# simon-donike/NIR-GAN

Measured on AMD Instinct MI355X. Metric: 256x256 RGB tiles/sec (G+D fwd+bwd+step), higher is better.
Workload: dtype f32 (3xbf16 split, 6 products, f32 accumulate) for the contractions with 32-channel runs incl. the Winograd plane GEMMs; exact f32 MFMA for the first / last layers; f32 everywhere else; 1 GPU; configs[1]: 6-block ResnetGenerator + 3-layer PatchGAN, bs=16/GPU, 256x256, GAN+L1, padding=0, fp32-equivalent MFMA (three bf16 terms, six products); global_batch=16, parallelism=dp1

## Files before the change

nir-gan_amd/csrc/igemm_wgrad.hip:

```cpp
#include "igemm_tiles.h"
#include "igemm_tile256.h"
#include "igemm_x3.h"
#include <cstdlib>

namespace {

template <int TN, int PREC = 0>
__global__ __launch_bounds__(256, 2) void wgrad_igemm_kernel(const ng::WgradParams p) {
    __shared__ __attribute__((aligned(16))) char st0[32 * (TN + 128) * 4];
    __shared__ __attribute__((aligned(16))) char st1[32 * (TN + 128) * 4];
    ng::wgrad_tile<TN, PREC>(p, blockIdx.x, st0, st1);
}

__global__ __launch_bounds__(256, 2) void wgrad_persist_kernel(const ng::WgradParams p) {
    __shared__ __attribute__((aligned(16))) char lds[65536];
    ng::wgrad_persist(p, blockIdx.x, gridDim.x, lds);
}

__global__ __launch_bounds__(256, 2) void wgrad_igemm16_kernel(const ng::WgradParams p) {
    __shared__ __attribute__((aligned(16))) char st0[32768];
    __shared__ __attribute__((aligned(16))) char st1[32768];
    ng::wgrad_tile16(p, blockIdx.x, st0, st1);
}


template <int PREC = 0, bool WB16 = false, bool AB16 = false, bool TW16 = false>
__global__ __launch_bounds__(256, 2) void conv_wgrad_pair_kernel(const ng::ConvParams cp, const ng::WgradParams wp, const int conv_blocks) {
    __shared__ __attribute__((aligned(16))) char st0[32768];
    __shared__ __attribute__((aligned(16))) char st1[32768];
    if (int(blockIdx.x) < conv_blocks)
        ng::conv_tile<128, PREC, WB16, AB16>(cp, blockIdx.x, st0, st1);
    else if constexpr (TW16)
        ng::wgrad_tile16(wp, int(blockIdx.x) - conv_blocks, st0, st1);
    else
        ng::wgrad_tile<128, PREC>(wp, int(blockIdx.x) - conv_blocks, st0, st1);
}

__global__ __launch_bounds__(512, 2) void wgrad_igemm256_kernel(const ng::WgradParams p, const int units) {
    __shared__ __attribute__((aligned(16))) char lds[ng::T256_LDS];
    bool again = false;
    for (int u = ng_xcd_remap(blockIdx.x, gridDim.x); u < units; u += gridDim.x) {
        if (again) ng::t256_bar();
        ng::wgrad_tile256(p, u, lds);
        again = true;
    }
}

__global__ __launch_bounds__(512, 2) void conv_wgrad_pair256_kernel(const ng::ConvParams cp, const ng::WgradParams wp, const int conv_wgs,
                                                                     const int conv_tiles, const int wgrad_units) {
    __shared__ __attribute__((aligned(16))) char lds[ng::T256_LDS];
    bool again = false;
    if (int(blockIdx.x) < conv_wgs) {
        for (int t = ng_xcd_remap(blockIdx.x, conv_wgs); t < conv_tiles; t += conv_wgs) {
            if (again) ng::t256_bar();
            ng::conv_tile256(cp, t, lds);
            again = true;
        }
    } else {
        const int y = int(gridDim.x) - conv_wgs;
        for (int u = ng_xcd_remap(int(blockIdx.x) - conv_wgs, y); u < wgrad_units; u += y) {
            if (again) ng::t256_bar();
            ng::wgrad_tile256(wp, u, lds);
            again = true;
        }
    }
}

template <int TN>
__global__ __launch_bounds__(512, 2) void wgrad_x3_kernel(const ng::WgradParams p, const int units) {
    __shared__ __attribute__((aligned(16))) char sP0[3 * 32 * TN * 2];
    __shared__ __attribute__((aligned(16))) char sP1[3 * 32 * TN * 2];
    __shared__ __attribute__((aligned(16))) char sQ0[3 * 32 * 256];
    __shared__ __attribute__((aligned(16))) char sQ1[3 * 32 * 256];
    for (int u = ng_xcd_remap(blockIdx.x, gridDim.x); u < units; u += gridDim.x) {
        ng::wgrad_tile_x3<TN>(p, u, sP0, sP1, sQ0, sQ1);
        __syncthreads();
    }
}

__global__ __launch_bounds__(256) void reduce_rows_kernel(const float* __restrict__ slabs, int nsplit, int N, int K,
                                                          const int32_t* __restrict__ map, float* __restrict__ dst,
                                                          int64_t dst_elems, int dst_row_stride, int accumulate, int row0) {
    __shared__ f32x4 part[4][64];
    const int lane = threadIdx.x & 63, grp = threadIdx.x >> 6;
    const int k4 = (blockIdx.x * 64 + lane) * 4;
    const int n = blockIdx.y;
    const size_t total = size_t(N) * K;
    f32x4 s = {0.f, 0.f, 0.f, 0.f};
    if (k4 < K) {
        const float* src = slabs + size_t(row0 + n) * K + k4;
        f32x4 s1 = {0.f, 0.f, 0.f, 0.f}, s2 = {0.f, 0.f, 0.f, 0.f}, s3 = {0.f, 0.f, 0.f, 0.f};
        int sp = grp;
        for (; sp + 12 < nsplit; sp += 16) {
            s += *reinterpret_cast<const f32x4*>(src + sp * total);
            s1 += *reinterpret_cast<const f32x4*>(src + (sp + 4) * total);
            s2 += *reinterpret_cast<const f32x4*>(src + (sp + 8) * total);
            s3 += *reinterpret_cast<const f32x4*>(src + (sp + 12) * total);
        }
        for (; sp < nsplit; sp += 4) s += *reinterpret_cast<const f32x4*>(src + sp * total);
        s = (s + s1) + (s2 + s3);
    }
    part[grp][lane] = s;
    __syncthreads();
    if (grp != 0 || k4 >= K) return;
    s = (part[0][lane] + part[1][lane]) + (part[2][lane] + part[3][lane]);
#pragma unroll
    for (int j = 0; j < 4; ++j) {
        const int mk = map[k4 + j];
        if (mk < 0) continue;
        const int64_t o = int64_t(n) * dst_row_stride + mk;
        if (o < dst_elems) dst[o] = accumulate ? dst[o] + s[j] : s[j];
    }
}

__global__ __launch_bounds__(256) void reduce_rows_batch_kernel(const long long* __restrict__ jobs, int njobs) {
    __shared__ f32x4 part[4][256];
    __shared__ float tile[64 * 16];
    int j = 0;
    for (int i = 1; i < njobs; ++i)
        if (int(blockIdx.x) >= int(jobs[i * 10 + 8])) j = i;
    const long long* J = jobs + j * 10;
    const float* slabs = reinterpret_cast<const float*>(J[0]);
    float* dst = reinterpret_cast<float*>(J[1]);
    const int32_t* map = reinterpret_cast<const int32_t*>(J[2]);
    const int nsplit = int(J[3]), N = int(J[4]), K = int(J[5]);
    const long long dst_elems = J[6];
    const int dst_row_stride = int(J[7] & 0xffffffffll), accumulate = int(J[7] >> 32);
    const int taps = int(J[9]);
    const int local = int(blockIdx.x) - int(J[8]);
    const int lane = threadIdx.x & 63, grp = threadIdx.x >> 6;
    const size_t total = size_t(N) * K;
    auto sum_splits = [&](const float* src) {
        f32x4 s = {0.f, 0.f, 0.f, 0.f}, s1 = {0.f, 0.f, 0.f, 0.f}, s2 = {0.f, 0.f, 0.f, 0.f}, s3 = {0.f, 0.f, 0.f, 0.f};
        int sp = grp;
        for (; sp + 12 < nsplit; sp += 16) {
            s += *reinterpret_cast<const f32x4*>(src + sp * total);
            s1 += *reinterpret_cast<const f32x4*>(src + (sp + 4) * total);
            s2 += *reinterpret_cast<const f32x4*>(src + (sp + 8) * total);
            s3 += *reinterpret_cast<const f32x4*>(src + (sp + 12) * total);
        }
        for (; sp < nsplit; sp += 4) s += *reinterpret_cast<const f32x4*>(src + sp * total);
        return (s + s1) + (s2 + s3);
    };
    if (taps > 0) {
        const int cin = K / taps, cb = cin >> 6;
        const int n = local / cb, c0 = (local - n * cb) << 6;
        const int nf = taps * 16;
        for (int f = lane; f < nf; f += 64) {
            const int t = f >> 4, q = f & 15;
            part[grp][f] = sum_splits(slabs + size_t(n) * K + t * cin + c0 + q * 4);
        }
        __syncthreads();
        for (int f = threadIdx.x; f < nf; f += 256) {
            const int t = f >> 4, q = f & 15;
            const f32x4 v = (part[0][f] + part[1][f]) + (part[2][f] + part[3][f]);
#pragma unroll
            for (int e = 0; e < 4; ++e) tile[(q * 4 + e) * taps + t] = v[e];
        }
        __syncthreads();
        float* drow = dst + (long long)n * dst_row_stride + (long long)c0 * taps;
        for (int i = threadIdx.x; i < 64 * taps; i += 256) drow[i] = accumulate ? drow[i] + tile[i] : tile[i];
        return;
    }
    const int kblocks = (K + 255) / 256;
    const int n = local / kblocks, kb = local - n * kblocks;
    const int k4 = (kb * 64 + lane) * 4;
    f32x4 s = {0.f, 0.f, 0.f, 0.f};
    if (k4 < K) s = sum_splits(slabs + size_t(n) * K + k4);
    part[grp][lane] = s;
    __syncthreads();
    if (grp != 0 || k4 >= K) return;
    s = (part[0][lane] + part[1][lane]) + (part[2][lane] + part[3][lane]);
#pragma unroll
    for (int q = 0; q < 4; ++q) {
        const int mk = map[k4 + q];
        if (mk < 0) continue;
        const long long o = (long long)n * dst_row_stride + mk;
        if (o < dst_elems) dst[o] = accumulate ? dst[o] + s[q] : s[q];
    }
}

typedef __bf16 bf16x4_t __attribute__((ext_vector_type(4)));

__device__ __forceinline__ void pack_store(float* dst, size_t elem, f32x4 v, int bf16) {
    if (bf16) *reinterpret_cast<bf16x4_t*>(reinterpret_cast<unsigned short*>(dst) + elem) = __builtin_convertvector(v, bf16x4_t);
    else *reinterpret_cast<f32x4*>(dst + elem) = v;
}

__global__ __launch_bounds__(256) void pack_rows_kernel(const float* __restrict__ src, int64_t src_elems, int src_row_stride,
                                                        const int32_t* __restrict__ map, float* __restrict__ dst, int N, int K, int bf16) {
    const int k4 = (blockIdx.x * 256 + threadIdx.x) * 4;
    const int n = blockIdx.y;
    if (k4 >= K) return;
    f32x4 v = {0.f, 0.f, 0.f, 0.f};
#pragma unroll
    for (int j = 0; j < 4; ++j) {
        const int mk = map[k4 + j];
        if (mk >= 0) {
            const int64_t o = int64_t(n) * src_row_stride + mk;
            if (o < src_elems) v[j] = src[o];
        }
    }
    pack_store(dst, size_t(n) * K + k4, v, bf16);
}

__global__ __launch_bounds__(256) void pack_rows_batch_kernel(const long long* __restrict__ jobs, int njobs) {
    int j = 0;
    for (int i = 1; i < njobs; ++i)
        if (int(blockIdx.x) >= int(jobs[i * 10 + 7])) j = i;
    const long long* J = jobs + j * 10;
    const float* src = reinterpret_cast<const float*>(J[0]);
    float* dst = reinterpret_cast<float*>(J[1]);
    const int32_t* map = reinterpret_cast<const int32_t*>(J[2]);
    const long long src_elems = J[3];
    const int K = int(J[5]), stride = int(J[6] & 0xffffffffll), bf16 = int(J[6] >> 32);
    const int kblocks = (K + 1023) / 1024;
    const int local = int(blockIdx.x) - int(J[7]);
    const int n = local / kblocks, kb = local - n * kblocks;
    const int k4 = (kb * 256 + threadIdx.x) * 4;
    if (k4 >= K) return;
    f32x4 v = {0.f, 0.f, 0.f, 0.f};
#pragma unroll
    for (int q = 0; q < 4; ++q) {
        const int mk = map[k4 + q];
        if (mk >= 0) {
            const long long o = (long long)n * stride + mk;
            if (o < src_elems) v[q] = src[o];
        }
    }
    pack_store(dst, size_t(n) * K + k4, v, bf16);
    if (J[8] != 0) {
        unsigned short* w3 = reinterpret_cast<unsigned short*>(J[8]) + size_t(n) * K + k4;
        const long long plane = J[9];
        typedef unsigned u32x2 __attribute__((ext_vector_type(2)));
        u32x2 h, m, l;
#pragma unroll
        for (int i = 0; i < 2; ++i) {
            const float x0 = v[2 * i], x1 = v[2 * i + 1];
            h[i] = ng::x3_pk(x0, x1);
            const float r0 = x0 - __builtin_bit_cast(float, h[i] << 16), r1 = x1 - __builtin_bit_cast(float, h[i] & 0xffff0000u);
            m[i] = ng::x3_pk(r0, r1);
            l[i] = ng::x3_pk(r0 - __builtin_bit_cast(float, m[i] << 16), r1 - __builtin_bit_cast(float, m[i] & 0xffff0000u));
        }
        *reinterpret_cast<u32x2*>(w3) = h;
        *reinterpret_cast<u32x2*>(w3 + plane) = m;
        *reinterpret_cast<u32x2*>(w3 + 2 * plane) = l;
    }
}

}


static int ng_cu_count() {
    static int cus = 0;
    if (cus == 0) {
        int dev = 0, n = 0;
        if (hipGetDevice(&dev) != hipSuccess || hipDeviceGetAttribute(&n, hipDeviceAttributeMultiprocessorCount, dev) != hipSuccess || n <= 0) n = 256;
        cus = n;
    }
    return cus;
}

static int pair256_split(const int G, const int conv_tiles, const int conv_nk, const int units, const int unit_nk) {
    int best = 1;
    long long best_cost = -1;
    for (int x = 1; x < G; ++x) {
        const long long c = (long long)((conv_tiles + x - 1) / x) * (conv_nk * 10 + 65), w = (long long)((units + (G - x) - 1) / (G - x)) * (unit_nk * 12 + 40);
        const long long cost = c > w ? c : w;
        if (best_cost < 0 || cost < best_cost) { best_cost = cost; best = x; }
    }
    return best;
}

enum WgradKernel { WGRAD_X3_TN256, WGRAD_X3_TN128, WGRAD_TILE256, WGRAD_PERSIST, WGRAD_TILE16, WGRAD_TILE_TN128, WGRAD_TILE_TN64 };
static const char* const WGRAD_KERNEL_NAMES[] = {"wgrad_x3_kernel<256>", "wgrad_x3_kernel<128>", "wgrad_igemm256_kernel", "wgrad_persist_kernel",
                                                 "wgrad_igemm16_kernel", "wgrad_igemm_kernel<128>", "wgrad_igemm_kernel<64>"};
struct WgradRoute { WgradKernel k; int units, grid; };
static WgradRoute wgrad_route(ng::WgradParams& p, const int algo) {
    const int G = ng_cu_count();
    if (p.prec == 3) {
        if (ng::wgrad_x3_ok(p)) {
            const int tn = ng::wgrad_x3_tn(p);
            const int units = (p.N / tn) * ((p.K + 127) >> 7) * p.nsplit * p.nplanes;
            return {tn == 256 ? WGRAD_X3_TN256 : WGRAD_X3_TN128, units, units < G ? units : G};
        }
        p.prec = 0;
    }
    if (algo == 0 && ng::wgrad_tile256_ok(p)) {
        const int units = (p.N >> 8) * (p.K >> 8) * p.nsplit;
        return {WGRAD_TILE256, units, units < G ? units : G};
    }
    const int tiles = p.ntiles_n * p.ntiles_k * p.nsplit * p.nplanes;
    if (ng::wgrad_persist_ok(p) && ng::wgrad_matrix_form(p) && tiles > 512 && algo != NIRGAN_WGRAD_ONE_UNIT) return {WGRAD_PERSIST, tiles, 512};
    if (p.pq_bf16) return {WGRAD_TILE16, tiles, tiles};
    return {p.N > 64 ? WGRAD_TILE_TN128 : WGRAD_TILE_TN64, tiles, tiles};
}

extern "C" int nirgan_wgrad_igemm(const nirgan_wgrad_desc* d, void* stream) {
    ng::WgradParams p;
    const int rc = ng::build_wgrad_params(d, p);
    if (rc != NIRGAN_OK) return rc;
    hipStream_t st = static_cast<hipStream_t>(stream);
    const WgradRoute r = wgrad_route(p, d->algo);
    const dim3 grid(r.grid);
    switch (r.k) {
        case WGRAD_X3_TN256: hipLaunchKernelGGL(wgrad_x3_kernel<256>, grid, dim3(512), 0, st, p, r.units); return nirgan_check_launch("wgrad_igemm (three-term split tile)");
        case WGRAD_X3_TN128: hipLaunchKernelGGL(wgrad_x3_kernel<128>, grid, dim3(512), 0, st, p, r.units); return nirgan_check_launch("wgrad_igemm (three-term split tile)");
        case WGRAD_TILE256: hipLaunchKernelGGL(wgrad_igemm256_kernel, grid, dim3(512), 0, st, p, r.units); return nirgan_check_launch("wgrad_igemm (256 x 256 tile)");
        case WGRAD_PERSIST: hipLaunchKernelGGL(wgrad_persist_kernel, grid, dim3(256), 0, st, p); break;
        case WGRAD_TILE16: hipLaunchKernelGGL(wgrad_igemm16_kernel, grid, dim3(256), 0, st, p); break;
        case WGRAD_TILE_TN128:
            if (p.prec == 0) hipLaunchKernelGGL((wgrad_igemm_kernel<128, 0>), grid, dim3(256), 0, st, p);
            else if (p.prec == 1) hipLaunchKernelGGL((wgrad_igemm_kernel<128, 1>), grid, dim3(256), 0, st, p);
            else hipLaunchKernelGGL((wgrad_igemm_kernel<128, 2>), grid, dim3(256), 0, st, p);
            break;
        case WGRAD_TILE_TN64:
            if (p.prec == 0) hipLaunchKernelGGL((wgrad_igemm_kernel<64, 0>), grid, dim3(256), 0, st, p);
            else if (p.prec == 1) hipLaunchKernelGGL((wgrad_igemm_kernel<64, 1>), grid, dim3(256), 0, st, p);
            else hipLaunchKernelGGL((wgrad_igemm_kernel<64, 2>), grid, dim3(256), 0, st, p);
            break;
    }
    return nirgan_check_launch("wgrad_igemm");
}

extern "C" const char* nirgan_wgrad_kernel_name(const nirgan_wgrad_desc* d) {
    ng::WgradParams p;
    if (ng::build_wgrad_params(d, p) != NIRGAN_OK) return nullptr;
    return WGRAD_KERNEL_NAMES[wgrad_route(p, d->algo).k];
}

enum PairKernel { PAIR_TWO_LAUNCHES, PAIR_TILE256, PAIR_TILE128 };
static const char* const PAIR_KERNEL_NAMES[] = {"(two launches)", "conv_wgrad_pair256_kernel", "conv_wgrad_pair_kernel"};
static PairKernel pair_route(const ng::ConvParams& cp, const ng::WgradParams& wp, const int w_algo) {
    if (cp.N <= 64 || wp.N <= 64 || cp.ksplit > 1 || (wp.pq_bf16 && !cp.in_bf16) || cp.prec == 3 || wp.prec == 3) return PAIR_TWO_LAUNCHES;
    if (cp.prec == 1 && cp.algo != NIRGAN_CONV_TILE128 && w_algo != NIRGAN_WGRAD_TILE128 && ng_cu_count() >= 2 && ng::conv_tile256_ok(cp, true, ng_cu_count())
        && ng::wgrad_tile256_ok(wp)) return PAIR_TILE256;
    return PAIR_TILE128;
}

extern "C" int nirgan_conv_wgrad_pair(const nirgan_conv_desc* c, const nirgan_wgrad_desc* w, void* stream) {
    ng::ConvParams cp;
    ng::WgradParams wp;
    int rc = ng::build_conv_params(c, cp);
    if (rc != NIRGAN_OK) return rc;
    rc = ng::build_wgrad_params(w, wp);
    if (rc != NIRGAN_OK) return rc;
    const PairKernel k = pair_route(cp, wp, w->algo);
    if (k == PAIR_TWO_LAUNCHES) {
        rc = nirgan_conv_igemm(c, stream);
        return rc != NIRGAN_OK ? rc : nirgan_wgrad_igemm(w, stream);
    }
    NG_REQUIRE(cp.prec == wp.prec, "conv_wgrad_pair: both halves must use the same precision");
    hipStream_t st = static_cast<hipStream_t>(stream);
    if (k == PAIR_TILE256) {
        const int conv_tiles = ((cp.M + 255) >> 8) * (cp.N >> 8), units = (wp.N >> 8) * (wp.K >> 8) * wp.nsplit, G = ng_cu_count();
        const int conv_wgs = pair256_split(G, conv_tiles, cp.ntaps * (cp.run >> 6), units, wp.rows_per_split >> 6);
        hipLaunchKernelGGL(conv_wgrad_pair256_kernel, dim3(G), dim3(512), 0, st, cp, wp, conv_wgs, conv_tiles, units);
        return nirgan_check_launch("conv_wgrad_pair (256 x 256 tiles)");
    }
    const int conv_blocks = cp.mtiles * cp.ntiles;
    const int wgrad_blocks = wp.ntiles_n * wp.ntiles_k * wp.nsplit;
    const dim3 grid(conv_blocks + wgrad_blocks);
    ng::conv_tile_form(cp, [&](auto form) {
        using F = decltype(form);
        if (F::ab16 && wp.pq_bf16) hipLaunchKernelGGL((conv_wgrad_pair_kernel<F::prec, F::wb16, F::ab16, F::ab16>), grid, dim3(256), 0, st, cp, wp, conv_blocks);
        else hipLaunchKernelGGL((conv_wgrad_pair_kernel<F::prec, F::wb16, F::ab16>), grid, dim3(256), 0, st, cp, wp, conv_blocks);
    });
    return nirgan_check_launch("conv_wgrad_pair");
}

extern "C" const char* nirgan_conv_wgrad_pair_kernel_name(const nirgan_conv_desc* c, const nirgan_wgrad_desc* w) {
    ng::ConvParams cp;
    ng::WgradParams wp;
    if (ng::build_conv_params(c, cp) != NIRGAN_OK || ng::build_wgrad_params(w, wp) != NIRGAN_OK) return nullptr;
    return PAIR_KERNEL_NAMES[pair_route(cp, wp, w->algo)];
}

extern "C" int nirgan_reduce_rows(const float* slabs, int nsplit, int N, int K, const int32_t* map,
                                  float* dst, int64_t dst_elems, int dst_row_stride, int accumulate, void* stream) {
    NG_REQUIRE(slabs && map && dst && nsplit >= 1 && N > 0 && K > 0 && K % 4 == 0 && N <= 65535, "reduce_rows: bad arguments");
    NG_REQUIRE(ng_aligned16(slabs), "reduce_rows: slabs must be 16-byte aligned");
    hipLaunchKernelGGL(reduce_rows_kernel, dim3((K + 255) / 256, N), dim3(256), 0, static_cast<hipStream_t>(stream),
                       slabs, nsplit, N, K, map, dst, dst_elems, dst_row_stride, accumulate, 0);
    return nirgan_check_launch("reduce_rows");
}

extern "C" int nirgan_reduce_rows_part(const float* slabs, int nsplit, int N, int row0, int rows, int K, const int32_t* map,
                                       float* dst, int64_t dst_elems, int dst_row_stride, int accumulate, void* stream) {
    NG_REQUIRE(slabs && map && dst && nsplit >= 1 && N > 0 && K > 0 && K % 4 == 0 && N <= 65535, "reduce_rows_part: bad arguments");
    NG_REQUIRE(row0 >= 0 && rows > 0 && row0 + rows <= N, "reduce_rows_part: rows [%d, %d) outside the slab's %d rows", row0, row0 + rows, N);
    NG_REQUIRE(ng_aligned16(slabs), "reduce_rows_part: slabs must be 16-byte aligned");
    hipLaunchKernelGGL(reduce_rows_kernel, dim3((K + 255) / 256, rows), dim3(256), 0, static_cast<hipStream_t>(stream),
                       slabs, nsplit, N, K, map, dst, dst_elems, dst_row_stride, accumulate, row0);
    return nirgan_check_launch("reduce_rows_part");
}

extern "C" int nirgan_reduce_rows_batch(const int64_t* jobs_device, int njobs, int total_blocks, void* stream) {
    NG_REQUIRE(jobs_device && njobs >= 1 && njobs <= 64 && total_blocks >= 1, "reduce_rows_batch: bad arguments");
    hipLaunchKernelGGL(reduce_rows_batch_kernel, dim3(total_blocks), dim3(256), 0, static_cast<hipStream_t>(stream),
                       reinterpret_cast<const long long*>(jobs_device), njobs);
    return nirgan_check_launch("reduce_rows_batch");
}

static int pack_rows_impl(const float* src, int64_t src_elems, int src_row_stride, const int32_t* map,
                          float* dst, int N, int K, int bf16, void* stream) {
    NG_REQUIRE(src && map && dst && N > 0 && K > 0 && K % 4 == 0 && N <= 65535, "pack_rows: bad arguments");
    NG_REQUIRE(ng_aligned16(dst), "pack_rows: dst must be 16-byte aligned");
    NG_REQUIRE(!bf16 || K % 8 == 0, "pack_rows: bf16 rows need K %% 8 == 0 (16-byte aligned rows)");
    hipLaunchKernelGGL(pack_rows_kernel, dim3((K + 1023) / 1024, N), dim3(256), 0, static_cast<hipStream_t>(stream),
                       src, src_elems, src_row_stride, map, dst, N, K, bf16);
    return nirgan_check_launch("pack_rows");
}

extern "C" int nirgan_pack_rows(const float* src, int64_t src_elems, int src_row_stride, const int32_t* map,
                                float* dst, int N, int K, void* stream) {
    return pack_rows_impl(src, src_elems, src_row_stride, map, dst, N, K, 0, stream);
}

extern "C" int nirgan_pack_rows_bf16(const float* src, int64_t src_elems, int src_row_stride, const int32_t* map,
                                     void* dst_bf16, int N, int K, void* stream) {
    return pack_rows_impl(src, src_elems, src_row_stride, map, static_cast<float*>(dst_bf16), N, K, 1, stream);
}

extern "C" int nirgan_pack_rows_batch(const int64_t* jobs_device, int njobs, int total_blocks, void* stream) {
    NG_REQUIRE(jobs_device && njobs >= 1 && njobs <= 256 && total_blocks >= 1, "pack_rows_batch: bad arguments");
    hipLaunchKernelGGL(pack_rows_batch_kernel, dim3(total_blocks), dim3(256), 0, static_cast<hipStream_t>(stream),
                       reinterpret_cast<const long long*>(jobs_device), njobs);
    return nirgan_check_launch("pack_rows_batch");
}
```

nir-gan_amd/csrc/igemm_x3.h:

```cpp
#pragma once
#include "igemm_tiles.h"

namespace ng {

constexpr int X3_A_TERM = 256 * 64;
constexpr int X3_A_BYTES = 3 * X3_A_TERM;

__device__ __forceinline__ int x3_key(const int row) { return (0x78 >> (2 * ((row >> 2) & 3))) & 3; }

__device__ __forceinline__ f32x4 ng_gld16_so(const char* base, unsigned off) {
    asm volatile("" : "+v"(off));
    return *reinterpret_cast<const NG_GLOBAL f32x4*>((const NG_GLOBAL char*)base + off);
}

typedef __bf16 bf16x2 __attribute__((ext_vector_type(2)));
typedef unsigned u32x4 __attribute__((ext_vector_type(4)));
__device__ __forceinline__ unsigned x3_pk(const float a, const float b) {
    const f32x2 v = {a, b};
    return __builtin_bit_cast(unsigned, __builtin_convertvector(v, bf16x2));
}
__device__ __forceinline__ float x3_sub(const float a, const float b) {
    float r;
    asm("v_sub_f32 %0, %1, %2" : "=v"(r) : "v"(a), "v"(b));
    return r;
// ... 123 lines not shown
        if (ct == L.ntaps) { ct = 0; cc += 32; }
    };
    f32x4 ra[4];
    auto loadA = [&]() {
        const int toff = __builtin_amdgcn_readlane(tapv, ct);
        const char* base = ng_uniform_ptr(L.in8 + (long long)(toff + cc) * 4);
        ra[0] = ng_gld16_so(base, a_goff[0]);
        ra[1] = ng_gld16_so(base, a_goff[0] + 16u);
        ra[2] = ng_gld16_so(base, a_goff[1]);
        ra[3] = ng_gld16_so(base, a_goff[1] + 16u);
    };
    auto issueB = [&](char* sB) {
#pragma unroll
        for (int i = 0; i < 3; ++i) {
            const int piece = wave + 8 * i;
            if (BN == 128 || piece < 3 * BPT) {
                const int term = piece / BPT;
                const char* base = ng_uniform_ptr(L.w8 + ((long long)term * L.w3_plane + ct * L.run + cc) * 2);
                ng_glds16_so(base, b_goff, sB + term * B_TERM + b_idx * 1024);
            }
        }
    };
    auto commitA = [&](char* sA, const int j) {
        bf16x8 H, M, Lo;
        x3_split8(ra[2 * j], ra[2 * j + 1], H, M, Lo);
        *reinterpret_cast<bf16x8*>(sA + a_wr[j]) = H;
        *reinterpret_cast<bf16x8*>(sA + X3_A_TERM + a_wr[j]) = M;
        *reinterpret_cast<bf16x8*>(sA + 2 * X3_A_TERM + a_wr[j]) = Lo;
    };

    f32x4 acc[4][NT];
    auto zero = [&]() {
#pragma unroll
        for (int mt = 0; mt < 4; ++mt)
#pragma unroll
            for (int nt = 0; nt < NT; ++nt) acc[mt][nt] = f32x4{0.f, 0.f, 0.f, 0.f};
    };
    const unsigned a_ad0 = unsigned(size_t((NG_LDS char*)sA0)) + unsigned(a_rd), a_ad1 = unsigned(size_t((NG_LDS char*)sA1)) + unsigned(a_rd);
    const unsigned b_ad0 = unsigned(size_t((NG_LDS char*)sB0)) + unsigned(b_rd), b_ad1 = unsigned(size_t((NG_LDS char*)sB1)) + unsigned(b_rd);
#define X3_DSR(dst, ad, off) asm volatile("ds_read_b128 %0, %1 offset:%2" : "=v"(dst) : "v"(ad), "n"(off) : "memory")
#define X3_RA(a, ad, MT) { X3_DSR(a[0], ad, (MT) * 1024); X3_DSR(a[1], ad, X3_A_TERM + (MT) * 1024); X3_DSR(a[2], ad, 2 * X3_A_TERM + (MT) * 1024); }
#define X3_RB(ad, NTI) { X3_DSR(B[NTI][0], ad, (NTI) * 1024); X3_DSR(B[NTI][1], ad, B_TERM + (NTI) * 1024); X3_DSR(B[NTI][2], ad, 2 * B_TERM + (NTI) * 1024); }
#define X3_WAIT(n) { asm volatile("s_waitcnt lgkmcnt(" #n ")" ::: "memory"); __builtin_amdgcn_sched_barrier(0); }
    auto compute = [&](const unsigned aad, const unsigned bad, auto more_tag, auto&& pre, auto&& mid) {
        constexpr bool MORE = decltype(more_tag)::value;
        bf16x8 B[NT][3], A[2][3];
        auto mma = [&](const int mt, const bf16x8 (&a)[3], const int nt) {
            f32x4 c = acc[mt][nt];
            c = __builtin_amdgcn_mfma_f32_16x16x32_bf16(a[2], B[nt][0], c, 0, 0, 0);
            c = __builtin_amdgcn_mfma_f32_16x16x32_bf16(a[0], B[nt][2], c, 0, 0, 0);
            c = __builtin_amdgcn_mfma_f32_16x16x32_bf16(a[1], B[nt][1], c, 0, 0, 0);
            c = __builtin_amdgcn_mfma_f32_16x16x32_bf16(a[1], B[nt][0], c, 0, 0, 0);
            c = __builtin_amdgcn_mfma_f32_16x16x32_bf16(a[0], B[nt][1], c, 0, 0, 0);
            c = __builtin_amdgcn_mfma_f32_16x16x32_bf16(a[0], B[nt][0], c, 0, 0, 0);
            acc[mt][nt] = c;
        };
        __builtin_amdgcn_sched_barrier(0);
        X3_RA(A[0], aad, 0)
        X3_RB(bad, 0)
        pre();
        __builtin_amdgcn_sched_barrier(0);
        if constexpr (NT == 4) {
            X3_RB(bad, 1) X3_WAIT(3) mma(0, A[0], 0); __builtin_amdgcn_sched_barrier(0);
            X3_RB(bad, 2) X3_WAIT(3) mma(0, A[0], 1); __builtin_amdgcn_sched_barrier(0);
            X3_RB(bad, 3) X3_WAIT(3) mma(0, A[0], 2); __builtin_amdgcn_sched_barrier(0);
            X3_RA(A[1], aad, 1) X3_WAIT(3) mma(0, A[0], 3); __builtin_amdgcn_sched_barrier(0);
        } else {
            X3_RB(bad, 1) X3_WAIT(3) mma(0, A[0], 0); __builtin_amdgcn_sched_barrier(0);
            X3_RA(A[1], aad, 1) X3_WAIT(3) mma(0, A[0], 1); __builtin_amdgcn_sched_barrier(0);
        }
        X3_RA(A[0], aad, 2) X3_WAIT(3)
#pragma unroll
        for (int nt = 0; nt < NT; ++nt) mma(1, A[1], nt);
        __builtin_amdgcn_sched_barrier(0);
        X3_RA(A[1], aad, 3) X3_WAIT(3)
        mid(0);
#pragma unroll
        for (int nt = 0; nt < NT; ++nt) mma(2, A[0], nt);
        __builtin_amdgcn_sched_barrier(0);
        if constexpr (MORE) { X3_WAIT(3) } else { X3_WAIT(0) }
        mid(1);
#pragma unroll
        for (int nt = 0; nt < NT; ++nt) mma(3, A[1], nt);
    };
#undef X3_WAIT
#undef X3_RB
#undef X3_RA
#undef X3_DSR
    constexpr int ESTORES = 2 * (32 / (64 / (CW / 4)));
    auto step = [&](const int cur, char* nA, char* nB, const bool more, const bool behind_stores = false) {
        if (behind_stores) {
            if constexpr (ESTORES == 16) asm volatile("s_waitcnt vmcnt(16)" ::: "memory");
            else asm volatile("s_waitcnt vmcnt(8)" ::: "memory");
        } else {
            asm volatile("s_waitcnt vmcnt(0)" ::: "memory");
        }
        __syncthreads();
        const unsigned aad = cur == 0 ? a_ad0 : a_ad1, bad = cur == 0 ? b_ad0 : b_ad1;
        if (more) {
            compute(aad, bad, std::true_type{}, [&]() { issueB(nB); loadA(); advance(); }, [&](const int j) { commitA(nA, j); });
        } else {
            compute(aad, bad, std::false_type{}, []() {}, [](const int) {});
        }
    };

    auto epilogue = [&]() -> bool {
        const NG_CONST ConvParams& p = *E.p;
        const int pM = p.M, pN = p.N, OHW = p.OHW, OW = p.OW, OH = p.OHW / p.OW, out_img = p.out_img, out_row = p.out_row * p.out_stride,
                  out_px = p.out_cs * p.out_stride, out_org = p.out_org, f_img = p.f_img, f_row = p.f_row * p.out_stride, f_px = p.ch * p.out_stride,
                  f_org = p.f_org, pC = p.ch, span = p.N / p.ch;
        const float* const f_y = p.f_y;
        const int mbase = E.m0 + wr * 64;
        const bool full = E.m0 + 256 <= pM;
        if (p.stats != nullptr && mbase < pM) {
            const int b = mbase / OHW;
            float* sp = p.stats + (size_t(b) * p.stats_cps + p.stats_chunk0 + ((mbase - b * OHW) >> 6) * span) * 4 * pC;
#pragma unroll
            for (int nt = 0; nt < NT; ++nt) {
                const float k0 = __shfl(acc[0][nt][0], lane & 15, 64);
                float s1 = 0.f, s2 = 0.f;
#pragma unroll
                for (int mt = 0; mt < 4; ++mt)
#pragma unroll
                    for (int r = 0; r < 4; ++r) {
                        const float v = acc[mt][nt][r] - k0;
                        s1 += v;
                        s2 += v * v;
                    }
                s1 += __shfl_xor(s1, 16, 64);
                s2 += __shfl_xor(s2, 16, 64);
                s1 += __shfl_xor(s1, 32, 64);
                s2 += __shfl_xor(s2, 32, 64);
                int col = E.n0 + wc * CW + nt * 16 + (lane & 15);
                if (col >= pC) col += 3 * pC;
                if (lane < 16) {
                    sp[col] = k0;
                    sp[pC + col] = s1;
                    sp[2 * pC + col] = s2;
                    sp[3 * pC + col] = 64.f;
                }
            }
        }
        constexpr int LPR = CW / 4, RPP = 64 / LPR;
        constexpr int SWM = CW / 16 - 1;
        const int sw_wr = ((lane >> 4) & SWM) << 4;
        float* const stg = reinterpret_cast<float*>(wave < 6 ? sA1 + wave * 8192 : sB1 + (wave - 6) * 8192);
        const bool fused = f_y != nullptr;
        const float fneg = p.f_act == NIRGAN_ACT_RELU ? 0.f : (p.f_act == NIRGAN_ACT_LRELU ? p.f_slope : 1.f);
        const int chunk = lane % LPR, lrow = lane / LPR;
        const int n = E.n0 + wc * CW + chunk * 4;
        f32x4 bv = {0.f, 0.f, 0.f, 0.f};
        if (p.bias != nullptr) bv = *reinterpret_cast<const f32x4*>(p.bias + n);
        int m = mbase + lrow;
        const int mc = m < pM ? m : pM - 1;
        int b = mc / OHW;
        const int r0 = mc - b * OHW;
        int oh = r0 / OW, ow = r0 - oh * OW;
        const int fb = (mbase < pM ? mbase : pM - 1) / OHW;
        f32x4 fm = {0.f, 0.f, 0.f, 0.f}, fr = fm, s1 = fm, s2 = fm;
        const int nq = n >= pC ? 1 : 0, nc = n - nq * pC;
        if (fused) {
            fm = *reinterpret_cast<const f32x4*>(p.f_mean + size_t(fb) * pC + nc);
            fr = *reinterpret_cast<const f32x4*>(p.f_rstd + size_t(fb) * pC + nc);
        }
        auto halves = [&](auto full_tag) {
            constexpr bool FULL = decltype(full_tag)::value;
            constexpr int P = 32 / RPP;
#pragma unroll
            for (int h = 0; h < 2; ++h) {
#pragma unroll
                for (int q = 0; q < 2; ++q)
#pragma unroll
                    for (int nt = 0; nt < NT; ++nt)
#pragma unroll
                        for (int r = 0; r < 4; ++r) stg[(q * 16 + (lane >> 4) * 4 + r) * CW + ((nt * 16 + (lane & 15)) ^ sw_wr)] = acc[h * 2 + q][nt][r];
                int ooff[P];
                bool ok[P];
                f32x4 yv[P];
#pragma unroll
                for (int pass = 0; pass < P; ++pass) {
                    ok[pass] = FULL || m < pM;
                    ooff[pass] = b * out_img + oh * out_row + ow * out_px + out_org + n;
                    if (fused && ok[pass]) yv[pass] = *reinterpret_cast<const f32x4*>(f_y + (size_t(b) * f_img + size_t(oh) * f_row + size_t(ow) * f_px + f_org + n));
                    m += RPP;
                    ow += RPP;
                    while (ow >= OW) { ow -= OW; ++oh; }
                    while (oh >= OH) { oh -= OH; ++b; }
                }
#pragma unroll
                for (int pass = 0; pass < P; ++pass) {
                    if (ok[pass]) {
                        f32x4 v = *reinterpret_cast<const f32x4*>(stg + (pass * RPP + lrow) * CW + ((chunk * 4) ^ ((((pass * RPP + lrow) >> 2) & SWM) << 4)));
                        v += bv;
#ifdef NG_X3_NT_STORES
                        __builtin_nontemporal_store(v, reinterpret_cast<f32x4*>(E.out + ooff[pass]));
#else
                        *reinterpret_cast<f32x4*>(E.out + ooff[pass]) = v;
#endif
                        if (fused) {
                            const f32x4 z = (yv[pass] - fm) * fr;
#pragma unroll
                            for (int q = 0; q < 4; ++q) {
                                const float gz = z[q] > 0.f ? v[q] : v[q] * fneg;
                                s1[q] += gz;
                                s2[q] += gz * z[q];
                            }
                        }
                    }
                }
            }
        };
        if (full) halves(std::true_type{}); else halves(std::false_type{});
        if (fused) {
#pragma unroll
            for (int q = 0; q < 4; ++q)
#pragma unroll
                for (int o = LPR; o < 64; o <<= 1) {
                    s1[q] += __shfl_xor(s1[q], o, 64);
                    s2[q] += __shfl_xor(s2[q], o, 64);
                }
            f32x4* const red = reinterpret_cast<f32x4*>(sRed);
            if (lane < LPR) {
                red[(wave * LPR + chunk) * 2] = s1;
                red[(wave * LPR + chunk) * 2 + 1] = s2;
            }
            __syncthreads();
            if ((wr & 1) == 0 && lane < LPR && mbase < pM) {
                const f32x4 t1 = s1 + red[((wave + 2) * LPR + chunk) * 2], t2 = s2 + red[((wave + 2) * LPR + chunk) * 2 + 1];
                float* pp = p.f_part + (size_t(fb) * p.f_cps + p.f_chunk0 + ((mbase - fb * OHW) >> 7) * span + nq) * 2 * pC + nc;
                *reinterpret_cast<f32x4*>(pp) = t1;
                *reinterpret_cast<f32x4*>(pp + pC) = t2;
            }
            __syncthreads();
        }
        return full;
    };

    int item = blockIdx.x;
    if (item >= total) return;
    locate(item, L);
    if (L.nk < 0) return;
    begin();
    loadA();
    issueB(sB0);
    advance();
    commitA(sA0, 0);
    commitA(sA0, 1);
    bool behind = false;
    while (true) {
        zero();
        const int nk = L.nk;
        int k = 0;
        if (nk >= 2) {
            if (behind) step(0, sA1, sB1, true, true); else step(0, sA1, sB1, true);
            step(1, sA0, sB0, 2 < nk);
            k = 2;
        }
        for (; k + 2 <= nk; k += 2) {
            step(0, sA1, sB1, true);
            step(1, sA0, sB0, k + 2 < nk);
        }
        if (k < nk) step(0, sA1, sB1, false);
        E = L;
        item += G;
        bool more = wp->spread ? true : item < total;
        __syncthreads();
        if (more) {
            locate(item, L);
            more = L.nk >= 0;
        }
        if (more) {
            begin();
            loadA();
            issueB(sB0);
            advance();
        }
        behind = epilogue();
        if (!more) break;
        commitA(sA0, 0);
        commitA(sA0, 1);
    }
}

int ng_launch_conv_x3(const ConvParams* ps, int n, int bn, int nplanes, long long in_plane, long long w3_pstride, long long out_plane,
                      hipStream_t st, const char* what);
int ng_cu_count_conv();
enum X3Kernel { X3R_PLAIN, X3R_STATS, X3R_GENERIC, X3_N128, X3_N64 };
X3Kernel conv_x3_route(const ConvParams* ps, int n, int bn);

inline bool conv_x3_ok(const ConvParams& p) {
    if (!(p.prec == 3 && p.w3 != nullptr && p.off32 && p.ksplit == 1)) return false;
    if (p.run % 32 != 0 || p.N % 64 != 0 || p.in_bf16 || p.w_bf16 || p.out16 || p.f_y16) return false;
    if (((p.out_cs | p.out_org | p.out_row | p.out_img) & 3) != 0) return false;
    return (long long)p.N * p.K * 2 < (1ll << 32);
}
inline int conv_x3_tiles(const ConvParams& p, const int bn) { return ((p.M + 255) >> 8) * (p.N / bn); }
inline int conv_x3_bn(const ConvParams* ps, const int n, const int cus) {
    if (ps[0].N % 128 != 0) return 64;
    long long tiles = 0;
    for (int i = 0; i < n; ++i) tiles += conv_x3_tiles(ps[i], 128);
    return tiles * 4 >= 3ll * cus ? 128 : 64;
}

template <int TN>
__device__ __forceinline__ void wgrad_tile_x3(const WgradParams& p, const int unit, char* sP0, char* sP1, char* sQ0, char* sQ1) {
    static_assert(TN == 128 || TN == 256, "128 or 256 rows n per unit");
    constexpr int PRS = TN * 2;
    constexpr int P_TERM = 32 * PRS, Q_TERM = 32 * 256;
    constexpr int MT = TN / 64;
    constexpr int PT = TN / 128;
    const int tid = threadIdx.x, lane = tid & 63;
    const int wave = __builtin_amdgcn_readfirstlane(tid >> 6);
    const int wr = wave >> 1, wc = wave & 1;
    const int ntn = p.N / TN, ntj = (p.K + 127) >> 7;
    const int per_plane = ntn * ntj * p.nsplit;
    const int plane = unit / per_plane, u = unit - plane * per_plane;
    const int nt_ = u % ntn, rest = u / ntn;
    const int jt = rest % ntj, split = rest / ntj;
    const int n0 = nt_ * TN, j0 = jt * 128;
    const int mstart = split * p.rows_per_split;
    int mend = mstart + p.rows_per_split;
    mend = mend < p.M ? mend : p.M;
    const int nk = mend > mstart ? (mend - mstart + 31) >> 5 : 0;
    const float* const Pp = p.p + (long long)plane * p.p_plane;
    const float* const Qp = p.q + (long long)plane * p.q_plane;

    const int lrow = tid >> 4, lch = tid & 15;
    const int lkey = 2 * ((lrow & 3) | (((lrow >> 3) & 1) << 2));
    unsigned p_goff[PT], q_goff;
    int p_wr[PT], q_wr;
#pragma unroll
    for (int i = 0; i < PT; ++i) {
        p_goff[i] = unsigned(lrow * p.p_cs + i * 128 + lch * 8) * 4u;
        p_wr[i] = lrow * PRS + (((i * 16 + lch) ^ lkey) << 4);
    }
    {
        int J = j0 + lch * 8;
        J = J < p.K ? J : 0;
        const int t = J / p.run;
        q_goff = unsigned(lrow * p.q_stride * p.q_cs + p.tap_off[t] + (J - t * p.run)) * 4u;
        q_wr = lrow * 256 + ((lch ^ lkey) << 4);
    }
    int sb = __builtin_amdgcn_readfirstlane(mstart / p.OHW);
    int soh = __builtin_amdgcn_readfirstlane((mstart - sb * p.OHW) / p.OW);
    int sow = __builtin_amdgcn_readfirstlane(mstart - sb * p.OHW - soh * p.OW);
    f32x4 rp[PT][2], rq[2];
    int mcur = mstart;
    auto load = [&]() {
        const char* pb = ng_uniform_ptr(reinterpret_cast<const char*>(Pp + (size_t(sb) * p.p_img + size_t(soh) * p.p_row + sow * p.p_cs + p.p_org + n0)));
        const char* qb = ng_uniform_ptr(reinterpret_cast<const char*>(Qp + (size_t(sb) * p.q_img + size_t(soh) * p.q_stride * p.q_row + sow * p.q_stride * p.q_cs + p.q_org)));
        if (mcur + 32 <= mend) {
#pragma unroll
            for (int i = 0; i < PT; ++i) {
                rp[i][0] = ng_gld16_so(pb, p_goff[i]);
                rp[i][1] = ng_gld16_so(pb, p_goff[i] + 16u);
            }
            rq[0] = ng_gld16_so(qb, q_goff);
            rq[1] = ng_gld16_so(qb, q_goff + 16u);
        } else {
            const int last = mend - 1 - mcur, back = lrow > last ? lrow - last : 0;
            const f32x4 z4 = {0.f, 0.f, 0.f, 0.f};
#pragma unroll
            for (int i = 0; i < PT; ++i) {
                const unsigned o = p_goff[i] - unsigned(back * p.p_cs) * 4u;
                rp[i][0] = ng_gld16_so(pb, o);
                rp[i][1] = ng_gld16_so(pb, o + 16u);
                if (back) rp[i][0] = rp[i][1] = z4;
            }
            const unsigned o = q_goff - unsigned(back * p.q_stride * p.q_cs) * 4u;
            rq[0] = ng_gld16_so(qb, o);
            rq[1] = ng_gld16_so(qb, o + 16u);
            if (back) rq[0] = rq[1] = z4;
        }
        mcur += 32;
        sow += 32;
        if (sow >= p.OW) { sow = 0; ++soh; }
        if (soh >= p.OH) { soh = 0; ++sb; }
    };
    auto commit = [&](char* sP, char* sQ) {
        bf16x8 H, M, L;
#pragma unroll
        for (int i = 0; i < PT; ++i) {
            x3_split8(rp[i][0], rp[i][1], H, M, L);
            *reinterpret_cast<bf16x8*>(sP + p_wr[i]) = H;
            *reinterpret_cast<bf16x8*>(sP + P_TERM + p_wr[i]) = M;
            *reinterpret_cast<bf16x8*>(sP + 2 * P_TERM + p_wr[i]) = L;
        }
        x3_split8(rq[0], rq[1], H, M, L);
        *reinterpret_cast<bf16x8*>(sQ + q_wr) = H;
        *reinterpret_cast<bf16x8*>(sQ + Q_TERM + q_wr) = M;
        *reinterpret_cast<bf16x8*>(sQ + 2 * Q_TERM + q_wr) = L;
    };

    const int g = lane >> 4, q = (lane >> 2) & 3, pp = lane & 3;
    const int fl = 2 * (q | ((g & 1) << 2));
    int a_ad[MT], b_ad[4];
#pragma unroll
    for (int mt = 0; mt < MT; ++mt) a_ad[mt] = (8 * g + q) * PRS + ((((wr * MT + mt) * 2) | (pp >> 1)) ^ fl) * 16 + 8 * (pp & 1);
#pragma unroll
    for (int nt = 0; nt < 4; ++nt) b_ad[nt] = (8 * g + q) * 256 + ((((wc * 4 + nt) * 2) | (pp >> 1)) ^ fl) * 16 + 8 * (pp & 1);
    f32x4 acc[MT][4];
#pragma unroll
    for (int mt = 0; mt < MT; ++mt)
#pragma unroll
        for (int nt = 0; nt < 4; ++nt) acc[mt][nt] = f32x4{0.f, 0.f, 0.f, 0.f};
    auto frag = [&](const char* img, const int ad, const int rs) -> bf16x8 {
        const s16x4 lo = __builtin_amdgcn_ds_read_tr16_b64_v4i16((NG_LDS s16x4*)(img + ad));
        const s16x4 hi = __builtin_amdgcn_ds_read_tr16_b64_v4i16((NG_LDS s16x4*)(img + ad + 4 * rs));
        const s16x8 v = __builtin_shufflevector(lo, hi, 0, 1, 2, 3, 4, 5, 6, 7);
        return __builtin_bit_cast(bf16x8, v);
    };
    auto compute = [&](const char* sP, const char* sQ, auto&& mid) {
        bf16x8 B[4][3], A[2][3];
        auto readA = [&](const int mt, bf16x8 (&a)[3]) {
#pragma unroll
            for (int t = 0; t < 3; ++t) a[t] = frag(sP + t * P_TERM, a_ad[mt], PRS);
        };
        auto readB = [&](const int nt) {
#pragma unroll
            for (int t = 0; t < 3; ++t) B[nt][t] = frag(sQ + t * Q_TERM, b_ad[nt], 256);
        };
        auto mma = [&](const int mt, const bf16x8 (&a)[3], const int nt) {
            f32x4 c = acc[mt][nt];
            c = __builtin_amdgcn_mfma_f32_16x16x32_bf16(a[2], B[nt][0], c, 0, 0, 0);
            c = __builtin_amdgcn_mfma_f32_16x16x32_bf16(a[0], B[nt][2], c, 0, 0, 0);
            c = __builtin_amdgcn_mfma_f32_16x16x32_bf16(a[1], B[nt][1], c, 0, 0, 0);
            c = __builtin_amdgcn_mfma_f32_16x16x32_bf16(a[1], B[nt][0], c, 0, 0, 0);
            c = __builtin_amdgcn_mfma_f32_16x16x32_bf16(a[0], B[nt][1], c, 0, 0, 0);
            c = __builtin_amdgcn_mfma_f32_16x16x32_bf16(a[0], B[nt][0], c, 0, 0, 0);
            acc[mt][nt] = c;
        };
        __builtin_amdgcn_sched_barrier(0);
        readA(0, A[0]);
        readB(0);
        __builtin_amdgcn_sched_barrier(0);
#pragma unroll
        for (int nt = 0; nt < 4; ++nt) {
            if (nt + 1 < 4) readB(nt + 1); else readA(1, A[1]);
            __builtin_amdgcn_sched_barrier(0);
            mma(0, A[0], nt);
            __builtin_amdgcn_sched_barrier(0);
        }
        if constexpr (MT == 2) {
            mid();
        } else {
            readA(2, A[0]);
            __builtin_amdgcn_sched_barrier(0);
#pragma unroll
            for (int nt = 0; nt < 4; ++nt) mma(1, A[1], nt);
            __builtin_amdgcn_sched_barrier(0);
            readA(3, A[1]);
            mid();
#pragma unroll
            for (int nt = 0; nt < 4; ++nt) mma(2, A[0], nt);
        }
#pragma unroll
        for (int nt = 0; nt < 4; ++nt) mma(MT - 1, A[1], nt);
    };
    auto step = [&](const char* cP, const char* cQ, char* nP, char* nQ, const bool more) {
        __syncthreads();
        if (more) {
            load();
            compute(cP, cQ, [&]() { commit(nP, nQ); });
        } else {
            compute(cP, cQ, []() {});
        }
    };
    if (nk > 0) {
        load();
        commit(sP0, sQ0);
        int k = 0;
        for (; k + 2 <= nk; k += 2) {
            step(sP0, sQ0, sP1, sQ1, true);
            step(sP1, sQ1, sP0, sQ0, k + 2 < nk);
        }
        if (k < nk) step(sP0, sQ0, sP1, sQ1, false);
    }

    __syncthreads();
    char* const reg = wave < 3 ? sP0 + wave * (MT * 4096) : (wave < 6 ? sP1 + (wave - 3) * (MT * 4096) : (wave == 6 ? sQ0 : sQ1));
    float* const stg = reinterpret_cast<float*>(reg);
#pragma unroll
    for (int mt = 0; mt < MT; ++mt)
#pragma unroll
        for (int nt = 0; nt < 4; ++nt)
#pragma unroll
            for (int r = 0; r < 4; ++r) stg[(mt * 16 + (lane >> 4) * 4 + r) * 64 + nt * 16 + (lane & 15)] = acc[mt][nt][r];
    float* const slab = p.slabs + (size_t(plane) * p.nsplit + split) * p.N * p.K;
    const int chunk = lane & 15, srow = lane >> 4;
    const int jj = j0 + wc * 64 + chunk * 4;
    if (jj < p.K) {
        float* dst = slab + size_t(n0 + wr * (TN / 4) + srow) * p.K + jj;
#pragma unroll 4
        for (int pass = 0; pass < MT * 4; ++pass)
            *reinterpret_cast<f32x4*>(dst + size_t(pass * 4) * p.K) = *reinterpret_cast<const f32x4*>(stg + (pass * 4 + srow) * 64 + chunk * 4);
    }
}

inline bool wgrad_x3_ok(const WgradParams& p) {
    const bool matrix = p.ntaps == 1 && p.tap_off[0] == 0 && p.q_stride == 1 && p.OH == 1 && p.OW == p.M && p.fast32_bytes;
    if (!(p.prec == 3 && !p.pq_bf16 && (p.fast32 || matrix))) return false;
    if (p.nplanes > 1 && !matrix) return false;
    if (p.N % 128 != 0 || p.run % 8 != 0 || p.K % 4 != 0) return false;
    return true;
}
inline int wgrad_x3_tn(const WgradParams& p) { return p.N % 256 == 0 ? 256 : 128; }

}
```

Baseline: 1121 tiles/s.

## Prefetch two k-steps ahead in x3 wgrad tile with piecewise commit/reload

Restructures the x3 wgrad main loop so global loads for the k-step after next are issued right after each register piece is committed to LDS. This deepens the software pipeline, giving loads a full compute step to land. The partial-tail handling is precomputed once as p_back offsets and zeroing happens at commit time instead of at load time. Optional s_memtime instrumentation (NG_WGRAD_X3_STAMP) is also added, but it is compiled out by default.

```diff
diff --git a/nir-gan_amd/csrc/igemm_wgrad.hip b/nir-gan_amd/csrc/igemm_wgrad.hip
--- a/nir-gan_amd/csrc/igemm_wgrad.hip
+++ b/nir-gan_amd/csrc/igemm_wgrad.hip
@@ -323,6 +323,18 @@
     return nirgan_check_launch("wgrad_igemm");
 }
 
+#ifdef NG_WGRAD_X3_STAMP
+extern "C" int nirgan_wgrad_x3_stamps(unsigned long long* host, int n, int reset) {
+    if (hipDeviceSynchronize() != hipSuccess) return -1;
+    if (host != nullptr && hipMemcpyFromSymbol(host, HIP_SYMBOL(ng::ng_wgx3_stamps), size_t(n) * 8) != hipSuccess) return -1;
+    if (reset) {
+        void* dp = nullptr;
+        if (hipGetSymbolAddress(&dp, HIP_SYMBOL(ng::ng_wgx3_stamps)) != hipSuccess || hipMemset(dp, 0, sizeof(ng::ng_wgx3_stamps)) != hipSuccess) return -1;
+    }
+    return 0;
+}
+#endif
+
 extern "C" const char* nirgan_wgrad_kernel_name(const nirgan_wgrad_desc* d) {
     ng::WgradParams p;
     if (ng::build_wgrad_params(d, p) != NIRGAN_OK) return nullptr;
diff --git a/nir-gan_amd/csrc/igemm_x3.h b/nir-gan_amd/csrc/igemm_x3.h
--- a/nir-gan_amd/csrc/igemm_x3.h
+++ b/nir-gan_amd/csrc/igemm_x3.h
@@ -449,6 +449,30 @@
     return tiles * 4 >= 3ll * cus ? 128 : 64;
 }
 
+
+#ifdef NG_WGRAD_X3_STAMP
+static __device__ unsigned long long ng_wgx3_stamps[256 * 8 * 16];
+#define WGX3_T(v) { __builtin_amdgcn_sched_barrier(0); asm volatile("s_memtime %0\n\ts_waitcnt lgkmcnt(0)" : "=s"(v) :: "memory"); __builtin_amdgcn_sched_barrier(0); }
+#define WGX3_ADD(slot, a, b) st_sum[slot] += (b) - (a);
+#define WGX3_COUNT(slot) st_sum[slot] += 1;
+#define WGX3_NEWTILE st_head = false;
+#define WGX3_HEAD if (!st_head) { st_sum[1] += st_t2 - st_t1; st_head = true; }
+#define WGX3_BEGIN unsigned long long st_sum[10] = {}, st_begin, st_r0, st_prev, st_t1 = 0, st_t2 = 0, st_t3 = 0; bool st_head = true; \
+    asm volatile("s_memtime %0\n\ts_memrealtime %1\n\ts_waitcnt lgkmcnt(0)" : "=s"(st_begin), "=s"(st_r0) :: "memory"); st_prev = st_begin;
+#define WGX3_END { unsigned long long c1_, r1_; __builtin_amdgcn_sched_barrier(0); \
+    asm volatile("s_waitcnt vmcnt(0)\n\ts_memtime %0\n\ts_memrealtime %1\n\ts_waitcnt lgkmcnt(0)" : "=s"(c1_), "=s"(r1_) :: "memory"); \
+    st_sum[5] += c1_ - st_prev; st_sum[6] += c1_ - st_begin; st_sum[7] += r1_ - st_r0; st_sum[9] += 1; \
+    if (lane == 0 && blockIdx.x < 256) for (int i_ = 0; i_ < 10; ++i_) ng_wgx3_stamps[(blockIdx.x * 8 + wave) * 16 + i_] += st_sum[i_]; }
+#else
+#define WGX3_T(v)
+#define WGX3_ADD(slot, a, b)
+#define WGX3_COUNT(slot)
+#define WGX3_NEWTILE
+#define WGX3_HEAD
+#define WGX3_BEGIN
+#define WGX3_END
+#endif
+
 template <int TN>
 __device__ __forceinline__ void wgrad_tile_x3(const WgradParams& p, const int unit, char* sP0, char* sP1, char* sQ0, char* sQ1) {
     static_assert(TN == 128 || TN == 256, "128 or 256 rows n per unit");
@@ -474,13 +498,10 @@
 
     const int lrow = tid >> 4, lch = tid & 15;
     const int lkey = 2 * ((lrow & 3) | (((lrow >> 3) & 1) << 2));
-    unsigned p_goff[PT], q_goff;
-    int p_wr[PT], q_wr;
-#pragma unroll
-    for (int i = 0; i < PT; ++i) {
-        p_goff[i] = unsigned(lrow * p.p_cs + i * 128 + lch * 8) * 4u;
-        p_wr[i] = lrow * PRS + (((i * 16 + lch) ^ lkey) << 4);
-    }
+    unsigned p_goff, q_goff;
+    int p_wr, q_wr;
+    p_goff = unsigned(lrow * p.p_cs + lch * 8) * 4u;
+    p_wr = lrow * PRS + ((lch ^ lkey) << 4);
     {
         int J = j0 + lch * 8;
         J = J < p.K ? J : 0;
@@ -491,52 +512,51 @@
     int sb = __builtin_amdgcn_readfirstlane(mstart / p.OHW);
     int soh = __builtin_amdgcn_readfirstlane((mstart - sb * p.OHW) / p.OW);
     int sow = __builtin_amdgcn_readfirstlane(mstart - sb * p.OHW - soh * p.OW);
+    unsigned p_back, q_back;
+    {
+        const int last = mend - 1 - (mstart + (nk - 1) * 32), back = lrow > last ? lrow - last : 0;
+        p_back = unsigned(back * p.p_cs) * 4u;
+        q_back = unsigned(back * p.q_stride * p.q_cs) * 4u;
+    }
     f32x4 rp[PT][2], rq[2];
+#define WGX3_GLD2(d0, d1, off, base, imm0, imm1) { d0 = ng_gld16_so(base, off + imm0##u); d1 = ng_gld16_so(base, off + imm1##u); }
     int mcur = mstart;
-    auto load = [&]() {
-        const char* pb = ng_uniform_ptr(reinterpret_cast<const char*>(Pp + (size_t(sb) * p.p_img + size_t(soh) * p.p_row + sow * p.p_cs + p.p_org + n0)));
-        const char* qb = ng_uniform_ptr(reinterpret_cast<const char*>(Qp + (size_t(sb) * p.q_img + size_t(soh) * p.q_stride * p.q_row + sow * p.q_stride * p.q_cs + p.q_org)));
-        if (mcur + 32 <= mend) {
-#pragma unroll
-            for (int i = 0; i < PT; ++i) {
-                rp[i][0] = ng_gld16_so(pb, p_goff[i]);
-                rp[i][1] = ng_gld16_so(pb, p_goff[i] + 16u);
-            }
-            rq[0] = ng_gld16_so(qb, q_goff);
-            rq[1] = ng_gld16_so(qb, q_goff + 16u);
+    auto load_piece = [&](const int j) {
+        const bool part = mcur + 32 > mend;
+        if (j == 0) {
+            const char* qb = ng_uniform_ptr(reinterpret_cast<const char*>(Qp + (size_t(sb) * p.q_img + size_t(soh) * p.q_stride * p.q_row + sow * p.q_stride * p.q_cs + p.q_org)));
+            const unsigned o = q_goff - (part ? q_back : 0u);
+            WGX3_GLD2(rq[0], rq[1], o, qb, 0, 16)
         } else {
-            const int last = mend - 1 - mcur, back = lrow > last ? lrow - last : 0;
-            const f32x4 z4 = {0.f, 0.f, 0.f, 0.f};
-#pragma unroll
-            for (int i = 0; i < PT; ++i) {
-                const unsigned o = p_goff[i] - unsigned(back * p.p_cs) * 4u;
-                rp[i][0] = ng_gld16_so(pb, o);
-                rp[i][1] = ng_gld16_so(pb, o + 16u);
-                if (back) rp[i][0] = rp[i][1] = z4;
-            }
-            const unsigned o = q_goff - unsigned(back * p.q_stride * p.q_cs) * 4u;
-            rq[0] = ng_gld16_so(qb, o);
-            rq[1] = ng_gld16_so(qb, o + 16u);
-            if (back) rq[0] = rq[1] = z4;
-        }
-        mcur += 32;
-        sow += 32;
-        if (sow >= p.OW) { sow = 0; ++soh; }
-        if (soh >= p.OH) { soh = 0; ++sb; }
-    };
-    auto commit = [&](char* sP, char* sQ) {
+            const char* pb = ng_uniform_ptr(reinterpret_cast<const char*>(Pp + (size_t(sb) * p.p_img + size_t(soh) * p.p_row + sow * p.p_cs + p.p_org + n0)));
+            const unsigned o = p_goff - (part ? p_back : 0u);
+            if (j == 1) WGX3_GLD2(rp[0][0], rp[0][1], o, pb, 0, 16)
+            else WGX3_GLD2(rp[PT - 1][0], rp[PT - 1][1], o, pb, 512, 528)
+        }
+        if (j == PT) {
+            mcur += 32;
+            sow += 32;
+            if (sow >= p.OW) { sow = 0; ++soh; }
+            if (soh >= p.OH) { soh = 0; ++sb; }
+        }
+    };
+#undef WGX3_GLD2
+    auto load_all = [&]() {
+#pragma unroll
+        for (int j = 0; j <= PT; ++j) load_piece(j);
+    };
+    auto commit_piece = [&](const int j, char* sP, char* sQ, const bool last) {
+        const bool z = last && p_back != 0u;
+        const f32x4 z4 = {0.f, 0.f, 0.f, 0.f};
+        f32x4& r0 = j == 0 ? rq[0] : rp[j == 1 ? 0 : PT - 1][0];
+        f32x4& r1 = j == 0 ? rq[1] : rp[j == 1 ? 0 : PT - 1][1];
+        char* const dst = j == 0 ? sQ + q_wr : sP + p_wr + (j - 1) * 256;
+        const int term = j == 0 ? Q_TERM : P_TERM;
         bf16x8 H, M, L;
-#pragma unroll
-        for (int i = 0; i < PT; ++i) {
-            x3_split8(rp[i][0], rp[i][1], H, M, L);
-            *reinterpret_cast<bf16x8*>(sP + p_wr[i]) = H;
-            *reinterpret_cast<bf16x8*>(sP + P_TERM + p_wr[i]) = M;
-            *reinterpret_cast<bf16x8*>(sP + 2 * P_TERM + p_wr[i]) = L;
-        }
-        x3_split8(rq[0], rq[1], H, M, L);
-        *reinterpret_cast<bf16x8*>(sQ + q_wr) = H;
-        *reinterpret_cast<bf16x8*>(sQ + Q_TERM + q_wr) = M;
-        *reinterpret_cast<bf16x8*>(sQ + 2 * Q_TERM + q_wr) = L;
+        x3_split8(z ? z4 : r0, z ? z4 : r1, H, M, L);
+        *reinterpret_cast<bf16x8*>(dst) = H;
+        *reinterpret_cast<bf16x8*>(dst + term) = M;
+        *reinterpret_cast<bf16x8*>(dst + 2 * term) = L;
     };
 
     const int g = lane >> 4, q = (lane >> 2) & 3, pp = lane & 3;
@@ -604,24 +624,45 @@
 #pragma unroll
         for (int nt = 0; nt < 4; ++nt) mma(MT - 1, A[1], nt);
     };
-    auto step = [&](const char* cP, const char* cQ, char* nP, char* nQ, const bool more) {
+    WGX3_BEGIN
+    auto pieces = [&](char* nP, char* nQ, const bool last, auto reload) {
+        constexpr bool RELOAD = decltype(reload)::value;
+#pragma unroll
+        for (int j = 0; j <= PT; ++j) {
+            WGX3_T(st_t2) WGX3_HEAD
+#ifdef NG_WGRAD_X3_STAMP
+            {
+                const int behind = (RELOAD || j == 0) ? 2 * PT : (j == 1 ? 2 * (PT - 1) : 0);
+                if (behind == 4) asm volatile("s_waitcnt vmcnt(4)" ::: "memory");
+                else if (behind == 2) asm volatile("s_waitcnt vmcnt(2)" ::: "memory");
+                else asm volatile("s_waitcnt vmcnt(0)" ::: "memory");
+            }
+#endif
+            WGX3_T(st_t3) WGX3_ADD(2, st_t2, st_t3)
+            commit_piece(j, nP, nQ, last);
+            if (RELOAD) load_piece(j);
+        }
+    };
+    auto step = [&](const char* cP, const char* cQ, char* nP, char* nQ, const int ahead) {
         __syncthreads();
-        if (more) {
-            load();
-            compute(cP, cQ, [&]() { commit(nP, nQ); });
-        } else {
-            compute(cP, cQ, []() {});
-        }
+        WGX3_T(st_t1) WGX3_ADD(0, st_prev, st_t1) WGX3_NEWTILE
+        if (ahead >= 2) compute(cP, cQ, [&]() { pieces(nP, nQ, false, std::true_type{}); });
+        else if (ahead == 1) compute(cP, cQ, [&]() { pieces(nP, nQ, true, std::false_type{}); });
+        else compute(cP, cQ, []() {});
+        WGX3_T(st_prev) WGX3_ADD(3, st_t1, st_prev)
+        WGX3_COUNT(8)
     };
     if (nk > 0) {
-        load();
-        commit(sP0, sQ0);
+        load_all();
+        pieces(sP0, sQ0, nk == 1, std::false_type{});
+        if (nk > 1) load_all();
+        WGX3_T(st_prev) WGX3_ADD(4, st_begin, st_prev)
         int k = 0;
         for (; k + 2 <= nk; k += 2) {
-            step(sP0, sQ0, sP1, sQ1, true);
-            step(sP1, sQ1, sP0, sQ0, k + 2 < nk);
-        }
-        if (k < nk) step(sP0, sQ0, sP1, sQ1, false);
+            step(sP0, sQ0, sP1, sQ1, nk - 1 - k >= 2 ? 2 : 1);
+            step(sP1, sQ1, sP0, sQ0, nk - 2 - k >= 2 ? 2 : nk - 2 - k);
+        }
+        if (k < nk) step(sP0, sQ0, sP1, sQ1, 0);
     }
 
     __syncthreads();
@@ -642,7 +683,15 @@
         for (int pass = 0; pass < MT * 4; ++pass)
             *reinterpret_cast<f32x4*>(dst + size_t(pass * 4) * p.K) = *reinterpret_cast<const f32x4*>(stg + (pass * 4 + srow) * 64 + chunk * 4);
     }
-}
+    WGX3_END
+}
+#undef WGX3_T
+#undef WGX3_ADD
+#undef WGX3_COUNT
+#undef WGX3_NEWTILE
+#undef WGX3_HEAD
+#undef WGX3_BEGIN
+#undef WGX3_END
 
 inline bool wgrad_x3_ok(const WgradParams& p) {
     const bool matrix = p.ntaps == 1 && p.tap_off[0] == 0 && p.q_stride == 1 && p.OH == 1 && p.OW == p.M && p.fast32_bytes;
```

After: 1131 tiles/s (median of 6 runs). No clear change (+0.9%).
